# jcmgray/cotengra

Hardware: AMD Instinct MI355X
Metric: contracted FLOP/s (whole node), Sycamore n53 m20 sliced amplitude (higher is better)
Workload: dtype complex64; 1 GPU; Sycamore n53 m20 amplitude, sliced tree, one slice per step per GPU; network=examples/benchmarks/sycamore_n53_m20_s0_e0_pABCDCDAB.json, tree=sycamore_m20_native.json, width_log2=32, parallelism=slice-parallel x1, 1 RCCL reduce, arithmetic=fp16x2 stem pairs and long tiled steps + fp32 MFMA

## Files before the change

cotengra_amd/csrc/ctg_stem_impl.h:

```cpp
#pragma once
#include "ctg_common.h"

#include <cstdio>
#include <cstdlib>
#include <type_traits>


namespace ctg {

typedef float f32x16 __attribute__((ext_vector_type(16)));
typedef float f32x4 __attribute__((ext_vector_type(4)));

#ifdef CTG_STEM_BOUNDS
template <class AR>
__device__ unsigned long long ctg_stem_oob[2];
#endif

#ifdef CTG_STEM_TIMELINE
#define CTG_TL_TILES 256
template <class AR>
__device__ unsigned long long ctg_stem_tl[8][CTG_TL_TILES][6];
template <class AR>
__device__ int ctg_stem_tl_on;
#endif

namespace {

constexpr int SW = 8;
constexpr int BR1_CHUNKS = 2;

__device__ __forceinline__ f32x16 mfma(float a, float b, f32x16 c) {
    return __builtin_amdgcn_mfma_f32_32x32x2f32(a, b, c, 0, 0, 0);
}

__device__ __forceinline__ constexpr int rowmap(int t) { return (t & 3) + 8 * (t >> 2); }

__device__ __forceinline__ float flip(float v, unsigned mask) {
    return __builtin_bit_cast(float, __builtin_bit_cast(unsigned, v) ^ mask);
}

template <bool FRAG1>
__device__ __forceinline__ void load_b_planes(float* P, const c64* __restrict__ B, const int64_t* off, int K,
                                              int N, bool pack, int tid, bool vec = false) {
    const int LDB = K + 4;
    for (int e = tid; e < K * N; e += SW * 64) {
        const int k = e / N, n = e - k * N;
        const int h = vec ? (k >> 1) & 1 : k & 1;
        const int slot = vec ? (((k & 15) >> 2) << 1) | (k & 1) : (k & 15) >> 1;
        const int kp = FRAG1 ? (k & ~15) + h * 8 + slot : k;
        const c64 v = B[off[e]];
        P[n * LDB + kp] = v.re;
        P[(N + n) * LDB + kp] = v.im;
        if (pack) P[(2 * N + n) * LDB + kp] = -v.im;
    }
}


typedef __bf16 bf16x8 __attribute__((ext_vector_type(8)));
typedef unsigned u32x4 __attribute__((ext_vector_type(4)));
__device__ __forceinline__ constexpr int bf3_ta(int t) { return t < 3 ? 0 : (t == 5 ? 2 : 1); }
__device__ __forceinline__ constexpr int bf3_tb(int t) { return t == 1 || t == 4 ? 1 : (t == 2 ? 2 : 0); }

// ... 153 lines not shown
#endif

template <typename T>
__device__ __forceinline__ void settle(T& v) {
    asm volatile("" : "+v"(v));
}

#ifndef CTG_STEM_WS_DEPTH
#define CTG_STEM_WS_DEPTH 2
#endif
#ifndef CTG_STEM_DEPTH
#define CTG_STEM_DEPTH 2
#endif
template <class AR, bool PACK1, bool PACK2, int RT1_, int CS1, int NCH, int IT2_, bool BR1, int K2Q, bool VEC, bool BF3,
          bool RI2, bool ONE, int ITM, bool PACKM, bool XM, bool LM, bool WS>
__device__ __forceinline__ void stem2_body(const StemArgs& p) {
    constexpr bool TRI = ITM > 0;
    static_assert(!LM, "reserved (the limb intermediate was removed): kernel names stay 17 arguments long");
    static_assert(BF3 || !AR::fp16, "fp16 x 2: the 16-bit kernels only (its object has no fp32 products)");
    static_assert(!AR::fp16 || !TRI, "fp16 x 2: pairs and single steps");
    static_assert(!WS || (XM && !ONE && IT2_ > 0 && IT2_ <= 2 && (PACK1 || RT1_ == 1)), "specialised waves: a static 16-bit pair");
    constexpr int PW = WS ? 4 : SW;
    constexpr int RT1 = WS ? 2 * RT1_ : RT1_;
    constexpr int IT2 = WS ? 2 * IT2_ : IT2_;
    static_assert(!XM || (BF3 && !TRI && NCH > 0), "two-accumulator real part: bf16 x 3, static, no three-step tile");
    constexpr bool XM1 = XM && !PACK1 && !WS;
    constexpr bool XM2 = XM && !PACK2;
    static_assert(!TRI || (NCH > 0 && IT2 > 0 && !RI2 && !ONE && K2Q == 0), "three-step tile: static, X / Y form");
    static_assert(!ONE || (!PACK1 && !PACK2 && !RI2 && IT2 == 0 && K2Q == 0), "one step: >= 32 columns, nothing of step 2");
    static_assert(!PACK1 || CS1 == 1, "16 columns are one group");
    static_assert(!BR1 || NCH > 0, "B1 in registers needs the chunk count at compile time");
    static_assert(K2Q == 0 || PACK2 || IT2 == 1 || RI2, "B2 in registers: one column group per wave");
    static_assert(!RI2 || (!PACK2 && !BF3 && NCH > 0 && IT2 > 0), "row-interleaved step 2: fp32, >= 32 columns, static");
    constexpr int RTW = PW / CS1;
    constexpr bool STATIC = NCH > 0;
    extern __shared__ __attribute__((aligned(16))) char smem[];
    const int K1 = p.K1, N1 = p.N1, K2 = K2Q > 0 ? 4 * K2Q : p.K2, N2 = p.N2;
    const int LDB1 = K1 + 4, LDB2 = K2 + 4, LD2 = K2Q > 0 ? 4 * K2Q + 4 : p.ld2;
    const int PLANE = p.rows2 * LD2;
    const int KM = TRI ? p.KM : 0, NM = TRI ? p.NM : 0, LDM = TRI ? p.ldM : 0, LDBM = KM + 4;
    const int PLANEM = TRI ? p.rowsM * LDM : 0;
    const int PLANE1 = TRI ? PLANEM : PLANE;
    float* P1 = (float*)smem;
    float* PM = P1 + (PACK1 ? 3 : 2) * N1 * LDB1;
    float* P2 = PM + (TRI ? (PACKM ? 3 : 2) * NM * LDBM : 0);
    float* mid = P2 + (PACK2 ? 3 : 2) * N2 * LDB2;
    const int RP = 3 * LD2;
    auto ri_off = [&](int e) __attribute__((always_inline)) { return RI2 ? (e / LD2) * RP + e % LD2 : e; };
    int mid_floats = 2 * (PLANE > PLANEM ? PLANE : PLANEM);
    if constexpr (RI2) {
        mid_floats = 3 * PLANE;
        if constexpr (K2Q > 0) {
            mid = P2;
            const int p2f = 2 * N2 * LDB2;
            mid_floats = mid_floats > p2f ? mid_floats : p2f;
        }
    }
    const int ROW1 = bf3_row(K1, true), ROW2 = bf3_row(K2, false), ROWM = TRI ? bf3_row(KM, false) : 0;
    unsigned short* Q1 = (unsigned short*)smem;
    unsigned short* QM = Q1 + (PACK1 ? 3 : 2) * N1 * ROW1;
    unsigned short* Q2 = QM + (TRI ? (PACKM ? 3 : 2) * NM * ROWM : 0);
    if constexpr (BF3) mid = (float*)(Q2 + (PACK2 ? 3 : 2) * N2 * ROW2);
    int64_t* oc_s = (int64_t*)(mid + ((mid_floats + 1) & ~1));

    const int tid = threadIdx.x;
    const int lane = tid & 63;
    const int wave = __builtin_amdgcn_readfirstlane(tid >> 6);
    const int kk = lane >> 5;
    const int l31 = lane & 31;
    const bool producer = !WS || wave < PW;
    const int wave1 = WS ? (wave & (PW - 1)) : wave;
    const int wrt = wave1 / CS1;
    const int wcol = (wave1 % CS1) * 32;

    const int64_t z = (int64_t)p.z0 + blockIdx.y;
    const c64* __restrict__ A = (const c64*)p.A + (sload64(p.soffA + z * p.zsA) + z * p.zA);
    const c64* __restrict__ B1 = (const c64*)p.B1 + (sload64(p.soffB1 + z * p.zsB1) + z * p.zB1);
    const c64* __restrict__ B2 = (const c64*)p.B2 + (sload64(p.soffB2 + z * p.zsB2) + z * p.zB2);
    float* __restrict__ C = (float*)((c64*)p.C + (sload64(p.soffC + z * p.zsC) + z * p.zC));
    const c64* __restrict__ BM = TRI ? (const c64*)p.BM + (sload64(p.soffBM + z * p.zsBM) + z * p.zBM) : nullptr;

    int bf3_ex = 0;
    float* const bf3_red = (float*)(oc_s + (ONE ? N1 : N2));
    float h2_sa = 1.f;
    int h2_exa = 0;
    if constexpr (AR::fp16) {
        h2_exa = p.amax != nullptr ? h2_exponent_of(read_max(p.amax)) : 0;
        h2_exa = __builtin_amdgcn_readfirstlane(h2_exa);
        h2_sa = pow2f(-h2_exa);
    }
    float h2_st = 1.f;
    float h2_vmax = 0.f;
    if constexpr (BF3) {
        const int ex1 = bf3_operand_exponent<AR>(B1, p.b1_off, K1 * N1, tid, bf3_red);
        const int ex2 = ONE ? 0 : bf3_operand_exponent<AR>(B2, p.b2_off, K2 * N2, tid, bf3_red);
        int exm = 0;
        if constexpr (TRI) {
            exm = bf3_operand_exponent<AR>(BM, p.bm_off, KM * NM, tid, bf3_red);
            load_b_planes_bf3<AR, false>(QM, BM, p.bm_off, KM, NM, PACKM ? 3 : 2, tid, false, pow2f(-exm));
        }
        bf3_ex = ex1 + ex2 + exm;
        load_b_planes_bf3<AR, true>(Q1, B1, p.b1_off, K1, N1, PACK1 ? 3 : 2, tid, VEC, pow2f(-ex1));
        if constexpr (!ONE) load_b_planes_bf3<AR, false>(Q2, B2, p.b2_off, K2, N2, PACK2 ? 3 : 2, tid, false, pow2f(-ex2));
    } else {
        load_b_planes<true>(P1, B1, p.b1_off, K1, N1, PACK1, tid, VEC);
        if constexpr (!ONE) load_b_planes<false>(P2, B2, p.b2_off, K2, N2, PACK2, tid);
// ... 20 lines not shown
    }
    const unsigned sgn2 = kk ? 0x80000000u : 0u;
    const unsigned short* q1p;
    const unsigned short* q1q;
    const unsigned short* q2x;
    const unsigned short* q2y = nullptr;
    {
        const int h16 = l31 >> 4;
        if (PACK1) {
            q1p = Q1 + ((h16 ? 1 : 0) * N1 + (l31 & 15)) * ROW1 + kk * 24;
            q1q = Q1 + ((h16 ? 0 : 2) * N1 + (l31 & 15)) * ROW1 + kk * 24;
        } else {
            q1p = Q1 + (wcol + l31) * ROW1 + kk * 24;
            q1q = Q1 + (N1 + wcol + l31) * ROW1 + kk * 24;
        }
        if (PACK2) {
            const int plane = kk == 0 ? (h16 ? 1 : 0) : (h16 ? 0 : 2);
            q2x = Q2 + (plane * N2 + (l31 & 15)) * ROW2;
        } else {
            q2x = Q2 + ((kk ? 1 : 0) * N2 + l31) * ROW2;
            q2y = Q2 + ((kk ? 0 : 1) * N2 + l31) * ROW2;
        }
    }
    const float* b2x;
    const float* b2y = nullptr;
    if (PACK2) {
        const int n = l31 & 15, h = l31 >> 4;
        const int plane = kk == 0 ? (h ? 1 : 0) : (h ? 0 : 2);
        b2x = P2 + (plane * N2 + n) * LDB2;
    } else {
        b2x = P2 + ((kk ? 1 : 0) * N2 + l31) * LDB2;
        b2y = P2 + ((kk ? 0 : 1) * N2 + l31) * LDB2;
    }
    int mid_lane = 0;
    if constexpr (!ONE) {
        if (PACK1) mid_lane = ri_off((int)p.mid_col[l31 & 15]) + (l31 >> 4) * (RI2 ? LD2 : PLANE1) + ri_off((int)p.mid_row[4 * kk]);
        else mid_lane = ri_off((int)p.mid_col[wcol + l31]) + ri_off((int)p.mid_row[4 * kk]);
    }
    settle(mid_lane);
    int mid_o[4];
#pragma unroll
    for (int b = 0; b < 4; ++b) mid_o[b] = ONE ? 0 : ri_off((int)sload64(p.mid_row + (b < 2 ? 1 << b : 2 << b)));
    int mid_rt[RT1];
    int64_t one_rt[RT1];
#pragma unroll
    for (int m = 0; m < RT1; ++m) {
        mid_rt[m] = ONE ? 0 : __builtin_amdgcn_readfirstlane(ri_off((int)sload64(p.mid_row + 32 * (wrt + RTW * m))));
        one_rt[m] = ONE ? sload64(p.out_row + 32 * (wrt + RTW * m)) : 0;
    }
    const int64_t one_col = ONE ? p.out_col[wcol + l31] : 0;
    auto mid_t = [&](int t) __attribute__((always_inline)) {
        return ((t & 1) ? mid_o[0] : 0) + ((t & 2) ? mid_o[1] : 0) + ((t & 4) ? mid_o[2] : 0) + ((t & 8) ? mid_o[3] : 0);
    };
    int64_t out_lane = p.out_row[RI2 ? 2 * kk : 4 * kk];
    if (PACK2) out_lane += (l31 >> 4) ? p.out_row[1] : 0;
    settle(out_lane);
    int64_t out_o[4];
#pragma unroll
    for (int b = 0; b < 4; ++b) out_o[b] = sload64(p.out_row + (RI2 ? (b == 0 ? 1 : 2 << b) : (b < 2 ? 1 << b : 2 << b)));
    auto out_t = [&](int t) __attribute__((always_inline)) {
        return ((t & 1) ? out_o[0] : 0) + ((t & 2) ? out_o[1] : 0) + ((t & 4) ? out_o[2] : 0) + ((t & 8) ? out_o[3] : 0);
    };
    const int n_rtM = TRI ? p.rowsM >> 5 : 1;
    const unsigned short* qmx[TRI ? ITM : 1];
    const unsigned short* qmy[TRI ? ITM : 1];
    const float* bmx[TRI ? ITM : 1];
    const float* bmy[TRI ? ITM : 1];
    int m2_lane[TRI ? ITM : 1], m2_rt[TRI ? ITM : 1], am_row[TRI ? ITM : 1];
    int m2_o[4] = {0, 0, 0, 0};
    if constexpr (TRI) {
        const int h16 = l31 >> 4;
#pragma unroll
        for (int i = 0; i < ITM; ++i) {
            const int item = wave + SW * i;
            const int cg = item / n_rtM, rtm = item - cg * n_rtM;
            am_row[i] = (rtm * 32 + l31) * LDM;
            if (PACKM) {
                const int plane = kk == 0 ? (h16 ? 1 : 0) : (h16 ? 0 : 2);
                qmx[i] = QM + (plane * NM + (l31 & 15)) * ROWM;
                qmy[i] = nullptr;
                bmx[i] = PM + (plane * NM + (l31 & 15)) * LDBM;
// ... 20 lines not shown
    const int ri_cg = RI2 ? wave % p.ng2 : 0;
    const int ri_rt0 = RI2 ? wave / p.ng2 : 0;
    const int ri_rts = RI2 ? SW / p.ng2 : 0;
    const float* ri_b = P2 + (kk * N2 + ri_cg * 32 + l31) * LDB2;

    float alpha = 1.f, alpha2 = 1.f;
    {
        int e1 = bf3_ex < -126 ? -126 : (bf3_ex > 126 ? 126 : bf3_ex);
        int e2 = bf3_ex - e1;
        e2 = e2 < -126 ? -126 : (e2 > 126 ? 126 : e2);
        if (p.facA != nullptr) {
            const double f = (*p.facA) * (*p.facB1) * (*p.facB2) * (TRI ? *p.facBM : 1.0);
            alpha = (f == 0.0 && p.check_zero) ? 0.f : (float)(1.0 / f * (BF3 ? exp2((double)e1) : 1.0));
        } else if (BF3 && bf3_ex != 0) {
            alpha = pow2f(e1);
        }
        if (BF3 && e2 != 0) alpha2 = pow2f(e2);
    }
    const int h2_e0 = bf3_ex + h2_exa;
    auto h2_set_alpha = [&](int et) __attribute__((always_inline)) {
        const int E = h2_e0 + et;
        const int e1 = E < -126 ? -126 : (E > 126 ? 126 : E);
        int e2 = E - e1;
        e2 = e2 < -126 ? -126 : (e2 > 126 ? 126 : e2);
        alpha = pow2f(e1);
        alpha2 = pow2f(e2);
    };
    if constexpr (AR::fp16) h2_set_alpha(0);
    const bool scaled = AR::fp16 ? true : __builtin_amdgcn_readfirstlane(alpha != 1.f || alpha2 != 1.f);
    __syncthreads();

    f32x4 b1r[BR1 && !BF3 ? NCH * 2 : 1][2];
    f32x4 b2r[K2Q > 0 && !BF3 ? K2Q : 1][PACK2 ? 1 : 2];
    bf16x8 b1r3[BR1 && BF3 ? NCH : 1][3][2];
    if constexpr (BR1 && BF3) {
#pragma unroll
        for (int c = 0; c < NCH; ++c)
#pragma unroll
            for (int q = 0; q < 3; ++q) {
                b1r3[c][q][0] = *(const bf16x8*)(q1p + c * 48 + q * 8);
                b1r3[c][q][1] = *(const bf16x8*)(q1q + c * 48 + q * 8);
            }
    }
    if constexpr (BR1 && !BF3) {
#pragma unroll
        for (int q = 0; q < NCH * 2; ++q) {
            b1r[q][0] = *(const f32x4*)(b1p + (q >> 1) * 16 + (q & 1) * 4);
            b1r[q][1] = *(const f32x4*)(b1q + (q >> 1) * 16 + (q & 1) * 4);
        }
    }
    if constexpr (K2Q > 0 && RI2) {
#pragma unroll
        for (int q = 0; q < K2Q; ++q) b2r[q][0] = *(const f32x4*)(ri_b + 4 * q);
    }
    if constexpr (K2Q > 0 && !BF3 && !RI2) {
        const int cg0 = PACK2 ? 0 : wave / (p.rows2 >> 5);
#pragma unroll
        for (int q = 0; q < K2Q; ++q) {
            b2r[q][0] = *(const f32x4*)(b2x + cg0 * 32 * LDB2 + 4 * q);
            if (!PACK2) {
                b2r[q][1] = *(const f32x4*)(b2y + cg0 * 32 * LDB2 + 4 * q);
#pragma unroll
                for (int t = 0; t < 4; ++t) b2r[q][0][t] = flip(b2r[q][0][t], sgn2);
            }
        }
    }
    const int nch = STATIC ? NCH : (K1 >> 4);
    const int n_rt2 = p.rows2 >> 5;
    const int n_items = n_rt2 * p.ng2;
    const int64_t n_tiles = p.n_tiles;
    const int64_t tile0 = blockIdx.x, tile_step = gridDim.x;
    const int64_t my_tiles = (n_tiles - tile0 + tile_step - 1) / tile_step;
    const int64_t last_tile = tile0 + (my_tiles - 1) * tile_step;

    constexpr int GD = WS ? CTG_STEM_WS_DEPTH : ((NCH > 0 && CTG_STEM_DEPTH == 4 && ((RT1 * NCH) & 1) == 0) ? 4 : 2);
    c64 regs[GD][8];
    int64_t ig = tile0;
    int im = 0, ic = 0;
    int64_t pend0 = 0, pend1 = 0, pend2 = 0, pend3 = 0;
    bool pend_live = false;
    auto prep = [&](auto always_tag) __attribute__((always_inline)) {
        constexpr bool ALWAYS = decltype(always_tag)::value;
        pend_live = ALWAYS || ig < n_tiles;
        if (pend_live) {
            const int64_t g = ALWAYS ? (ig < last_tile ? ig : last_tile) : ig;
            const int64_t gh = g >> p.g_lo_shift, gl = g & (p.g_lo - 1);
            pend0 = sload64(p.gA_hi + uniform64(gh));
            pend1 = sload64(p.gA_lo + uniform64(gl));
            pend2 = sload64(p.rt_a + (wrt + RTW * im));
            pend3 = sload64(p.chunk_a + ic);
            if (++ic == nch) {
                ic = 0;
                if (++im == RT1) {
                    im = 0;
                    ig += tile_step;
                }
            }
        }
    };
    auto fire2 = [&](c64 (&r)[8], int q, int64_t base, auto always_tag) __attribute__((always_inline)) {
        if (decltype(always_tag)::value || pend_live) {
            if constexpr (XM) {
                typedef const __attribute__((address_space(1))) char* gptr;
                uint64_t u0 = (uint64_t)A + ((uint64_t)(base + kj[2 * q]) << 3);
                uint64_t u1 = (uint64_t)A + ((uint64_t)(base + kj[2 * q + 1]) << 3);
                asm volatile("" : "+s"(u0), "+s"(u1));
                settle(a_lane);
                const unsigned al = a_lane;
                if (VEC) {
                    const f32x4 v = *(const __attribute__((address_space(1))) f32x4*)((gptr)u0 + al);
                    r[2 * q] = c64{v[0], v[1]};
                    r[2 * q + 1] = c64{v[2], v[3]};
                } else {
                    typedef float f32x2 __attribute__((ext_vector_type(2)));
                    const f32x2 v0 = *(const __attribute__((address_space(1))) f32x2*)((gptr)u0 + al);
                    const f32x2 v1 = *(const __attribute__((address_space(1))) f32x2*)((gptr)u1 + al);
                    r[2 * q] = c64{v0[0], v0[1]};
                    r[2 * q + 1] = c64{v1[0], v1[1]};
                }
                return;
            }
            const char* sb = (const char*)(A + (base + kj[2 * q]));
#ifdef CTG_STEM_BOUNDS
            {
                const uint64_t lim = (uint64_t)p.a_elems * 8;
                const uint64_t o0 = (uint64_t)(sb + a_lane - (const char*)A);
// ... 43 lines not shown
        }
#endif
        *(float2*)q = v;
    };
    auto drain = [&](int lo, int hi, auto set_tag, auto scaled_tag) __attribute__((always_inline)) {
        constexpr int SET = decltype(set_tag)::value < NSET ? decltype(set_tag)::value : 0;
#pragma unroll
        for (int i = lo; i < hi; ++i) {
            if constexpr (RI2) {
                float2 v;
                v.x = cr[SET][i >> 3][2 * (i & 7)];
                v.y = cr[SET][i >> 3][2 * (i & 7) + 1];
                if constexpr (decltype(scaled_tag)::value) {
                    v.x = v.x * alpha * alpha2;
                    v.y = v.y * alpha * alpha2;
                }
                store2(pdst + 2 * out_t(i), v);
            } else {
                store2(pdst + 2 * out_t(PACK2 ? 2 * i : i), pv[i]);
            }
        }
    };
    auto consume = [&](c64 (&r)[8], int m, int ch, auto always_tag, auto drain_tag, auto scaled_tag)
                       __attribute__((always_inline)) {
        constexpr bool DRAIN = decltype(drain_tag)::value >= 0;
        const int64_t base = pend0 + pend1 + pend2 + pend3;
        if constexpr (BF3) {
            float re[8], im[8];
#pragma unroll
            for (int j = 0; j < 8; ++j) {
                re[j] = r[j].re;
                im[j] = r[j].im;
            }
            bf16x8 r3[3], i3[3], n3[3], bp3[3], bq3[3];
            AR::split(re, r3, h2_sa);
            AR::split(im, i3, h2_sa);
            __builtin_amdgcn_sched_barrier(0);
#pragma unroll
            for (int q = 0; q < 4; ++q) fire2(r, q, base, always_tag);
#pragma unroll
            for (int q = 0; q < 3; ++q) {
                if (!PACK1 && !XM1) n3[q] = __builtin_bit_cast(bf16x8, __builtin_bit_cast(u32x4, i3[q]) ^ 0x80008000u);
                if constexpr (BR1) {
                    bp3[q] = b1r3[ch][q][0];
                    bq3[q] = b1r3[ch][q][1];
                } else {
                    bp3[q] = *(const bf16x8*)(q1p + ch * 48 + q * 8);
                    bq3[q] = *(const bf16x8*)(q1q + ch * 48 + q * 8);
                }
            }
            __builtin_amdgcn_sched_barrier(0);
            const bool fresh = XM && STATIC && ch == 0;
            f32x16 zero16;
#pragma unroll
            for (int u = 0; u < 16; ++u) zero16[u] = 0.f;
#pragma unroll
            for (int t = 0; t < 6; t += AR::t_step(t)) {
                const int ta = bf3_ta(t), tb = bf3_tb(t);
                if (PACK1) {
                    ax[m] = AR::mfma(r3[ta], bp3[tb], (fresh && t == 0) ? zero16 : ax[m]);
                    ax[m] = AR::mfma(i3[ta], bq3[tb], ax[m]);
                } else if constexpr (XM1) {
                    ax[m] = AR::mfma(r3[ta], bp3[tb], (fresh && t == 0) ? zero16 : ax[m]);
                    ay[m] = AR::mfma(r3[ta], bq3[tb], (fresh && t == 0) ? zero16 : ay[m]);
                    axm[m] = AR::mfma(i3[ta], bq3[tb], (fresh && t == 0) ? zero16 : axm[m]);
                    ay[m] = AR::mfma(i3[ta], bp3[tb], ay[m]);
                } else {
                    ax[m] = AR::mfma(r3[ta], bp3[tb], (fresh && t == 0) ? zero16 : ax[m]);
                    ay[m] = AR::mfma(r3[ta], bq3[tb], (fresh && t == 0) ? zero16 : ay[m]);
                    ax[m] = AR::mfma(n3[ta], bq3[tb], ax[m]);
                    ay[m] = AR::mfma(i3[ta], bp3[tb], ay[m]);
                }
                __builtin_amdgcn_sched_barrier(0);
                if constexpr (DRAIN)
                    drain(AR::t_index(t) * NST / AR::products, (AR::t_index(t) + 1) * NST / AR::products, drain_tag, scaled_tag);
            }
            __builtin_amdgcn_sched_barrier(0);
            prep(always_tag);
            __builtin_amdgcn_sched_barrier(0);
            return;
        }
        f32x4 bp[2], bq[2];
        if constexpr (BR1) {
            bp[0] = b1r[ch * 2][0];
            bp[1] = b1r[ch * 2 + 1][0];
            bq[0] = b1r[ch * 2][1];
            bq[1] = b1r[ch * 2 + 1][1];
        } else {
            bp[0] = *(const f32x4*)(b1p + ch * 16);
            bq[0] = *(const f32x4*)(b1q + ch * 16);
            bp[1] = *(const f32x4*)(b1p + ch * 16 + 4);
            bq[1] = *(const f32x4*)(b1q + ch * 16 + 4);
        }
#pragma unroll
        for (int j = 0; j < 8; ++j) {
            const float re = r[j].re, im = r[j].im;
            const float p_ = bp[j >> 2][j & 3], q_ = bq[j >> 2][j & 3];
            __builtin_amdgcn_sched_barrier(0);
            if (PACK1) {
                ax[m] = mfma(re, p_, ax[m]);
                ax[m] = mfma(im, q_, ax[m]);
            } else {
                ax[m] = mfma(re, p_, ax[m]);
                ay[m] = mfma(re, q_, ay[m]);
                ax[m] = mfma(flip(im, sgn), q_, ax[m]);
                ay[m] = mfma(im, p_, ay[m]);
            }
            __builtin_amdgcn_sched_barrier(0);
            if (j & 1) fire2(r, j >> 1, base, always_tag);
            if constexpr (DRAIN) drain(j * NST / 8, (j + 1) * NST / 8, drain_tag, scaled_tag);
        }
        __builtin_amdgcn_sched_barrier(0);
        prep(always_tag);
        __builtin_amdgcn_sched_barrier(0);
    };
    auto zero_acc = [&](int m) __attribute__((always_inline)) {
        if constexpr (XM && STATIC) return;
#pragma unroll
        for (int t = 0; t < 16; ++t) {
            ax[m][t] = 0.f;
            if (!PACK1) ay[m][t] = 0.f;
            if constexpr (XM1) axm[m][t] = 0.f;
        }
    };
    auto scatter = [&]() __attribute__((always_inline)) {
#pragma unroll
        for (int m = 0; m < RT1; ++m) {
            float* dst = mid + (mid_lane + mid_rt[m]);
#pragma unroll
            for (int t = 0; t < 16; ++t) {
                dst[mid_t(t)] = XM1 ? ax[m][t] - axm[m][t] : ax[m][t];
                if constexpr (RI2) {
                    if constexpr (PACK1) {
                        if (l31 >> 4) dst[LD2 + mid_t(t)] = -ax[m][t];
                    } else {
                        dst[LD2 + mid_t(t)] = ay[m][t];
                        dst[2 * LD2 + mid_t(t)] = -ay[m][t];
                    }
                } else {
                    if (!PACK1) dst[PLANE1 + mid_t(t)] = ay[m][t];
                }
            }
        }
    };
    auto item_row = [&](int item, int64_t c_tile) __attribute__((always_inline)) -> int64_t {
        const int cg = item / n_rt2, rt2 = item - cg * n_rt2;
        int64_t c_row = c_tile + sload64(p.out_row + 32 * rt2);
        asm volatile("" : "+s"(c_row));
        return c_row;
    };
    auto item2r = [&](int rt2, int64_t c_row, auto set_tag, auto prev_tag, auto scaled_tag) __attribute__((always_inline)) {
        constexpr int SET = decltype(set_tag)::value;
        constexpr bool DRAIN = decltype(prev_tag)::value >= 0;
        const float* a0p = mid + ri_plane + (rt2 * 32 + (l31 >> 1)) * RP;
        const float* a1p = a0p + 16 * RP;
        const int64_t c_col = oc_s[ri_cg * 32 + l31];
        f32x4 a0[2], a1[2], bq[2];
        a0[0] = *(const f32x4*)(a0p);
        a1[0] = *(const f32x4*)(a1p);
        constexpr int NQ = K2Q > 0 ? K2Q : 1;
        if constexpr (K2Q > 0) {
// ... 192 lines not shown
            constexpr bool SC = decltype(scaled_tag)::value;
            pdst = C + 2 * (c_row + out_lane + c_col);
            if (PACK2) {
                const bool hi = (l31 >> 4) != 0;
#pragma unroll
                for (int t = 0; t < 16; t += 2) {
                    const float mine = hi ? cx[t] : cx[t + 1];
                    const float got = __builtin_bit_cast(
                        float, __builtin_amdgcn_ds_swizzle(__builtin_bit_cast(int, mine), 0x401F));
                    float2 v;
                    v.x = hi ? got : cx[t];
                    v.y = hi ? cx[t + 1] : got;
                    if (SC) {
                        v.x = v.x * alpha * alpha2;
                        v.y = v.y * alpha * alpha2;
                    }
                    if constexpr (BF3) h2_vmax = fmaxf(h2_vmax, fmaxf(fabsf(v.x), fabsf(v.y)));
                    pv[t >> 1] = v;
                }
            } else {
#pragma unroll
                for (int t = 0; t < 16; ++t) {
                    float2 v;
                    const float xr = XM2 ? cx[t] - cxm[t] : cx[t];
                    v.x = SC ? xr * alpha * alpha2 : xr;
                    v.y = SC ? cy[t] * alpha * alpha2 : cy[t];
                    if constexpr (BF3) h2_vmax = fmaxf(h2_vmax, fmaxf(fabsf(v.x), fabsf(v.y)));
                    pv[t] = v;
                }
            }
            if constexpr (!decltype(defer_tag)::value) drain(0, NST, std::integral_constant<int, 0>{}, scaled_tag);
        }
    };
    f32x16 mx[TRI ? ITM : 1], my[TRI ? ITM : 1];
    auto item_mid = [&](auto ii) __attribute__((always_inline)) {
        constexpr int I = decltype(ii)::value;
        f32x16 cx, cy;
#pragma unroll
        for (int t = 0; t < 16; ++t) {
            cx[t] = 0.f;
            cy[t] = 0.f;
        }
        const float* a_base = mid + kk * PLANEM + am_row[I];
        if constexpr (BF3) {
            for (int kb = 0; kb < (KM >> 3); ++kb) {
                const f32x4 lo = *(const f32x4*)(a_base + 8 * kb), hi = *(const f32x4*)(a_base + 8 * kb + 4);
                const float a8[8] = {lo[0], lo[1], lo[2], lo[3], hi[0], hi[1], hi[2], hi[3]};
                bf16x8 a3[3], ax3[3], bx3[3], by3[3];
                AR::split(a8, a3);
#pragma unroll
                for (int q = 0; q < 3; ++q) {
                    ax3[q] = PACKM ? a3[q]
                                   : __builtin_bit_cast(bf16x8, __builtin_bit_cast(u32x4, a3[q]) ^ (sgn2 | (sgn2 >> 16)));
                    bx3[q] = *(const bf16x8*)(qmx[I] + kb * 24 + q * 8);
                    if (!PACKM) by3[q] = *(const bf16x8*)(qmy[I] + kb * 24 + q * 8);
                }
#pragma unroll
                for (int t = 0; t < 6; t += AR::t_step(t)) {
                    cx = AR::mfma(ax3[bf3_ta(t)], bx3[bf3_tb(t)], cx);
                    if (!PACKM) cy = AR::mfma(a3[bf3_ta(t)], by3[bf3_tb(t)], cy);
                }
            }
        } else {
            const int nq = KM >> 2;
            f32x4 af[2], bx[2], by[2];
            af[0] = *(const f32x4*)(a_base);
// ... 51 lines not shown
            float mx = 0.f;
#pragma unroll
            for (int m = 0; m < RT1; ++m)
#pragma unroll
                for (int t = 0; t < 16; ++t) {
                    const float xr = XM1 ? ax[m][t] - axm[m][t] : ax[m][t];
                    mx = fmaxf(mx, fabsf(xr));
                    if (!PACK1) mx = fmaxf(mx, fabsf(ay[m][t]));
                }
#pragma unroll
            for (int o = 32; o > 0; o >>= 1) mx = fmaxf(mx, __shfl_xor(mx, o));
            if (lane == 0) bf3_red[h2_par * 8 + wave1] = mx;
            if constexpr (WS) h2_par ^= 1;
        }
    };
    auto h2_consume = [&]() __attribute__((always_inline)) {
        if constexpr (AR::fp16 && !ONE) {
            float mx = bf3_red[h2_par * 8];
#pragma unroll
            for (int w = 1; w < PW; ++w) mx = fmaxf(mx, bf3_red[h2_par * 8 + w]);
            const int et = __builtin_amdgcn_readfirstlane(h2_exponent_of(mx));
            h2_st = pow2f(-et);
            h2_set_alpha(et);
            h2_par ^= 1;
        }
    };
    auto tile_c = [&](int64_t g) __attribute__((always_inline)) -> int64_t {
        const int64_t gh = g >> p.g_lo_shift, gl = g & (p.g_lo - 1);
        return sload64(p.gC_hi + uniform64(gh)) + sload64(p.gC_lo + uniform64(gl));
    };

    auto run = [&](auto scaled_tag) __attribute__((always_inline)) {
    if constexpr (WS) {
        constexpr int NT = RT1 * NCH;
        constexpr int U = (NT % GD == 0) ? 1 : ((2 * NT) % GD == 0 ? 2 : 4);
        static_assert((U * NT) % GD == 0, "a pass of U tiles returns to gather set 0");
        auto step1 = [&](auto slot0_tag) __attribute__((always_inline)) {
            constexpr int SLOT0 = decltype(slot0_tag)::value;
            static_for<0, RT1>([&](auto mi) __attribute__((always_inline)) {
                constexpr int M = decltype(mi)::value;
                static_for<0, NCH>([&](auto ci) __attribute__((always_inline)) {
                    constexpr int CH = decltype(ci)::value;
                    consume(regs[(SLOT0 + M * NCH + CH) & (GD - 1)], M, CH, std::true_type{}, std::integral_constant<int, -1>{}, scaled_tag);
                });
            });
        };
        auto step2 = [&](int64_t gc) __attribute__((always_inline)) {
            const int64_t c_tile = tile_c(gc);
            int64_t c_rows[IT2];
            static_for<0, IT2>([&](auto ii) __attribute__((always_inline)) {
                c_rows[decltype(ii)::value] = item_row(wave1 + PW * decltype(ii)::value, c_tile);
            });
            static_for<0, IT2>([&](auto ii) __attribute__((always_inline)) {
                constexpr int I = decltype(ii)::value;
                item2(wave1 + PW * I, c_rows[I], scaled_tag, std::integral_constant<bool, (I > 0)>{}, std::true_type{});
            });
        };
        if (producer) {
            static_for<0, GD>([&](auto gi) __attribute__((always_inline)) { issue(regs[decltype(gi)::value], std::true_type{}); });
            prep(std::true_type{});
            step1(std::integral_constant<int, 0>{});
            for (int64_t t = 0; t < my_tiles; t += U) {
                static_for<0, U>([&](auto ui) __attribute__((always_inline)) {
                    constexpr int UI = decltype(ui)::value;
                    if (t + UI < my_tiles) {
                        h2_publish();
                        __syncthreads();
                        scatter();
                        __syncthreads();
                        if (t + UI + 1 < my_tiles) step1(std::integral_constant<int, ((UI + 1) * NT) & (GD - 1)>{});
                    }
                });
            }
        } else {
            for (int64_t t = 0; t < my_tiles; ++t) {
                __syncthreads();
                if (t > 0) drain(0, NST, std::integral_constant<int, 0>{}, scaled_tag);
                __syncthreads();
                h2_consume();
                step2(tile0 + t * tile_step);
            }
            drain(0, NST, std::integral_constant<int, 0>{}, scaled_tag);
// ... 496 lines not shown
    if (form == 3 && items == 2 * SW && p.N2 >= 32) form = 1;
    if (items >= 4 * SW) form = 0;
    return form;
}

template <class AR>
static void stem_kernel_name(const StemArgs& p, char* buf, size_t n) {
    const StemShape s = stem2_shape(p);
    const char* const kn = AR::kernel_name;
    auto tf = [](bool b) { return b ? "true" : "false"; };
    if (p.tri) {
        const Stem3Shape t = stem3_shape(p);
        snprintf(buf, n, "%s<%s,%s,%d,%d,%d,%d,%s,0,%s,%s,false,false,%d,%s>", kn, tf(t.p1), tf(t.p2), t.rt1, t.cs1,
                 t.nch, t.it2, tf(t.nch <= BR1_CHUNKS), tf(t.vec), tf(stem_wants_16bit(p)), t.itm, tf(t.pm));
        return;
    }
    if (p.one) {
        const bool st = stem1_static(s), b3 = stem2_bf3(p);
        if (st && b3)
            snprintf(buf, n, "%s<false,false,%d,%d,%d,0,%s,0,%s,true,false,true,0,false,true,false>", kn, s.rt1, s.cs1,
                     s.nch, tf(s.nch <= BR1_CHUNKS), tf(s.vec));
        else
            snprintf(buf, n, "%s<false,false,%d,%d,%d,0,%s,0,%s,%s,false,true>", kn, s.rt1, s.cs1, st ? s.nch : 0,
                     tf(st && (b3 ? s.nch <= BR1_CHUNKS : p.K1 <= 64)), tf(s.vec), tf(b3));
        return;
    }
    if (stem2_bf3(p)) {
        const int form = stem2_bf3_form<AR>(p);
        if (form == 0)
            snprintf(buf, n, "%s<%s,%s,%d,%d,%d,%d,%s,0,%s,true,false,false>", kn, tf(s.p1), tf(s.p2), s.rt1, s.cs1,
                     s.nch, s.it2, tf(s.nch <= BR1_CHUNKS), tf(s.vec));
        else
            snprintf(buf, n, "%s<%s,%s,%d,%d,%d,%d,%s,0,%s,true,false,false,0,false,true,false,%s>", kn, tf(s.p1), tf(s.p2),
                     s.rt1, s.cs1, s.nch, s.it2, tf(s.nch <= BR1_CHUNKS), tf(s.vec), tf(form >= 3));
    }
    else if (stem2_variant(p))
        snprintf(buf, n, "%s<%s,%s,%d,%d,%d,%d,%s,%d,%s,false,%s,false>", kn, tf(s.p1), tf(s.p2), s.rt1, s.cs1, s.nch,
                 s.it2, tf(s.br1), s.k2q, tf(s.vec), tf(s.ri2));
    else
        snprintf(buf, n, "%s<%s,%s,%d,%d,0,0,false,0,%s,false,false,false>", kn, tf(s.p1), tf(s.p2), s.rt1, s.cs1,
                 tf(s.vec));
}

static bool stem_uses_16bit(const StemArgs& p) { return !p.tri && stem2_supported_shape(p) && stem2_bf3(p); }

template <class AR>
static hipError_t launch_stem(const StemArgs& p, hipStream_t stream) {
    if (!stem2_supported_shape(p)) return hipErrorInvalidValue;
    if constexpr (AR::fp16) {
        if (!stem_uses_16bit(p)) return hipErrorInvalidValue;
    } else {
        if (p.tri) {
            const Stem3Shape t = stem3_shape(p);
            const bool b3 = stem_wants_16bit(p);
#define CTG_STEM_GO3T(A, M, B, R, CS, NC, IM, IT, V)                                                                  \
    if (t.p1 == A && t.pm == M && t.p2 == B && t.rt1 == R && t.cs1 == CS && t.nch == NC && t.itm == IM && t.it2 == IT && \
        t.vec == V)                                                                                                   \
        return b3 ? launch_stem3_t<A, M, B, R, CS, NC, IM, IT, V, true>(p, stream)                                    \
                  : launch_stem3_t<A, M, B, R, CS, NC, IM, IT, V, false>(p, stream);
            CTG_STEM_TRI(CTG_STEM_GO3T)
#undef CTG_STEM_GO3T
            return hipErrorInvalidValue;
        }
    }
    if (p.one) {
        const StemShape s = stem2_shape(p, true);
        const bool b3 = stem2_bf3(p);
        if (stem1_static(s)) {
#define CTG_STEM_GO1(R, CS, NC, V)                                                                            \
    if (s.rt1 == R && s.cs1 == CS && s.nch == NC && s.vec == V) {                                             \
        if (b3) return launch_stem1_t<AR, R, CS, NC, (NC <= BR1_CHUNKS), V, true>(p, stream);                 \
        if constexpr (!AR::fp16) return launch_stem1_t<AR, R, CS, NC, (NC <= 4), V, false>(p, stream);        \
    }
            CTG_STEM_ONE(CTG_STEM_GO1)
#undef CTG_STEM_GO1
        }
        if constexpr (!AR::fp16) {
#define CTG_STEM_CASE1(R, CS)                                                               \
    if (s.rt1 == R && s.cs1 == CS)                                                          \
        return s.vec ? launch_stem1_t<AR, R, CS, 0, false, true, false>(p, stream)          \
                     : launch_stem1_t<AR, R, CS, 0, false, false, false>(p, stream);
            CTG_STEM_CASE1(1, 1) CTG_STEM_CASE1(2, 1) CTG_STEM_CASE1(1, 2) CTG_STEM_CASE1(2, 2)
            CTG_STEM_CASE1(1, 4) CTG_STEM_CASE1(2, 4)
#undef CTG_STEM_CASE1
        }
        return hipErrorInvalidValue;
    }
    if (stem2_bf3(p)) {
        const StemShape s = stem2_shape(p, true);
        const int form = stem2_bf3_form<AR>(p);
#define CTG_STEM_GO3(P1, P2, R, CS, NC, IT, V)                                                                           \
    if (s.p1 == P1 && s.p2 == P2 && s.rt1 == R && s.cs1 == CS && s.nch == NC && s.it2 == IT && s.vec == V) {             \
        if constexpr (AR::max_form >= 3 && IT <= 2 && (P1 || R == 1) && (P2 || IT < 2)) {                                \
            if (form == 3)                                                                                               \
                return launch_stem2_t<AR, P1, P2, R, CS, NC, IT, (NC <= BR1_CHUNKS), 0, V, true, false, true, true>(p, stream);  \
        }                                                                                                                \
        if constexpr (IT < 4) {                                                                                          \
            if (form == 1)                                                                                               \
                return launch_stem2_t<AR, P1, P2, R, CS, NC, IT, (NC <= BR1_CHUNKS), 0, V, true, false, true, false>(p, stream); \
        } else {                                                                                                         \
            if (form == 0) return launch_stem2_t<AR, P1, P2, R, CS, NC, IT, (NC <= BR1_CHUNKS), 0, V, true>(p, stream);  \
        }                                                                                                                \
        return hipErrorInvalidValue;                                                                                     \
    }
        CTG_STEM_GEO(CTG_STEM_GO3)
#undef CTG_STEM_GO3
    }
    if constexpr (!AR::fp16) {
        const StemShape s = stem2_shape(p);
        if (stem2_variant(p)) {
#define CTG_STEM_GO(P1, P2, R, CS, NC, IT, B1, KQ, V, RI)                                              \
    if (s.p1 == P1 && s.p2 == P2 && s.rt1 == R && s.cs1 == CS && s.nch == NC && s.it2 == IT && s.br1 == B1 && \
        s.k2q == KQ && s.vec == V && s.ri2 == RI)                                                      \
        return launch_stem2_t<AR, P1, P2, R, CS, NC, IT, B1, KQ, V, false, RI>(p, stream);
            CTG_STEM_INST(CTG_STEM_GO)
#undef CTG_STEM_GO
        }
#define CTG_STEM_CASE(P1, P2, R, CS)                                                                    \
    if (s.p1 == P1 && s.p2 == P2 && s.rt1 == R && s.cs1 == CS)                                          \
        return s.vec ? launch_stem2_t<AR, P1, P2, R, CS, 0, 0, false, 0, true>(p, stream)               \
                     : launch_stem2_t<AR, P1, P2, R, CS, 0, 0, false, 0, false>(p, stream);
#define CTG_STEM_CASES(P2)             \
    CTG_STEM_CASE(true, P2, 1, 1)      \
    CTG_STEM_CASE(true, P2, 2, 1)      \
    CTG_STEM_CASE(false, P2, 1, 1)     \
    CTG_STEM_CASE(false, P2, 2, 1)     \
    CTG_STEM_CASE(false, P2, 1, 2)     \
    CTG_STEM_CASE(false, P2, 2, 2)     \
// ... 13 lines not shown
```

Measured before the change: 161400 billion FLOP/s.

## Share A fragments across column groups in specialised-wave stem and add K-chunked step-2 path

In the warp-specialised 16-bit stem pair, when several column groups exist each wave now covers all column groups of a row tile. The split A fragment is reused across column groups instead of being recomputed per wave, and B1 register residency is sized to match. A new step-2 routine (item2k) handles two column groups per wave with the A fragments kept in registers and B chunks double-buffered. The aim is to cut redundant A splitting and LDS reads, at the cost of more registers per wave and possible occupancy or spill pressure.

```diff
diff --git a/cotengra_amd/csrc/ctg_stem_impl.h b/cotengra_amd/csrc/ctg_stem_impl.h
--- a/cotengra_amd/csrc/ctg_stem_impl.h
+++ b/cotengra_amd/csrc/ctg_stem_impl.h
@@ -28,6 +28,7 @@
 
 constexpr int SW = 8;
 constexpr int BR1_CHUNKS = 2;
+constexpr bool stem_br1_ws(int cs1, int nch) { return (cs1 == 2 ? 2 : 1) * nch <= BR1_CHUNKS; }
 
 __device__ __forceinline__ f32x16 mfma(float a, float b, f32x16 c) {
     return __builtin_amdgcn_mfma_f32_32x32x2f32(a, b, c, 0, 0, 0);
@@ -247,7 +248,10 @@
     static_assert(!BR1 || NCH > 0, "B1 in registers needs the chunk count at compile time");
     static_assert(K2Q == 0 || PACK2 || IT2 == 1 || RI2, "B2 in registers: one column group per wave");
     static_assert(!RI2 || (!PACK2 && !BF3 && NCH > 0 && IT2 > 0), "row-interleaved step 2: fp32, >= 32 columns, static");
-    constexpr int RTW = PW / CS1;
+    constexpr bool SH1 = WS && CS1 > 1 && RT1 % CS1 == 0;
+    constexpr int CG1 = SH1 ? CS1 : 1;
+    constexpr int RR1 = RT1 / CG1;
+    constexpr int RTW = SH1 ? PW : PW / CS1;
     constexpr bool STATIC = NCH > 0;
     extern __shared__ __attribute__((aligned(16))) char smem[];
     const int K1 = p.K1, N1 = p.N1, K2 = K2Q > 0 ? 4 * K2Q : p.K2, N2 = p.N2;
@@ -285,8 +289,8 @@
     const int l31 = lane & 31;
     const bool producer = !WS || wave < PW;
     const int wave1 = WS ? (wave & (PW - 1)) : wave;
-    const int wrt = wave1 / CS1;
-    const int wcol = (wave1 % CS1) * 32;
+    const int wrt = SH1 ? wave1 : wave1 / CS1;
+    const int wcol = SH1 ? 0 : (wave1 % CS1) * 32;
 
     const int64_t z = (int64_t)p.z0 + blockIdx.y;
     const c64* __restrict__ A = (const c64*)p.A + (sload64(p.soffA + z * p.zsA) + z * p.zA);
@@ -373,12 +377,16 @@
         b2x = P2 + ((kk ? 1 : 0) * N2 + l31) * LDB2;
         b2y = P2 + ((kk ? 0 : 1) * N2 + l31) * LDB2;
     }
-    int mid_lane = 0;
-    if constexpr (!ONE) {
-        if (PACK1) mid_lane = ri_off((int)p.mid_col[l31 & 15]) + (l31 >> 4) * (RI2 ? LD2 : PLANE1) + ri_off((int)p.mid_row[4 * kk]);
-        else mid_lane = ri_off((int)p.mid_col[wcol + l31]) + ri_off((int)p.mid_row[4 * kk]);
-    }
-    settle(mid_lane);
+    int mid_lane[CG1];
+#pragma unroll
+    for (int cg = 0; cg < CG1; ++cg) {
+        mid_lane[cg] = 0;
+        if constexpr (!ONE) {
+            if (PACK1) mid_lane[cg] = ri_off((int)p.mid_col[l31 & 15]) + (l31 >> 4) * (RI2 ? LD2 : PLANE1) + ri_off((int)p.mid_row[4 * kk]);
+            else mid_lane[cg] = ri_off((int)p.mid_col[wcol + 32 * cg + l31]) + ri_off((int)p.mid_row[4 * kk]);
+        }
+        settle(mid_lane[cg]);
+    }
     int mid_o[4];
 #pragma unroll
     for (int b = 0; b < 4; ++b) mid_o[b] = ONE ? 0 : ri_off((int)sload64(p.mid_row + (b < 2 ? 1 << b : 2 << b)));
@@ -386,8 +394,8 @@
     int64_t one_rt[RT1];
 #pragma unroll
     for (int m = 0; m < RT1; ++m) {
-        mid_rt[m] = ONE ? 0 : __builtin_amdgcn_readfirstlane(ri_off((int)sload64(p.mid_row + 32 * (wrt + RTW * m))));
-        one_rt[m] = ONE ? sload64(p.out_row + 32 * (wrt + RTW * m)) : 0;
+        mid_rt[m] = ONE ? 0 : __builtin_amdgcn_readfirstlane(ri_off((int)sload64(p.mid_row + 32 * (wrt + RTW * (m / CG1)))));
+        one_rt[m] = ONE ? sload64(p.out_row + 32 * (wrt + RTW * (m / CG1))) : 0;
     }
     const int64_t one_col = ONE ? p.out_col[wcol + l31] : 0;
     auto mid_t = [&](int t) __attribute__((always_inline)) {
@@ -474,15 +482,18 @@
 
     f32x4 b1r[BR1 && !BF3 ? NCH * 2 : 1][2];
     f32x4 b2r[K2Q > 0 && !BF3 ? K2Q : 1][PACK2 ? 1 : 2];
-    bf16x8 b1r3[BR1 && BF3 ? NCH : 1][3][2];
+    bf16x8 b1r3[CG1][BR1 && BF3 ? NCH : 1][3][2];
+    const int q1cg = 32 * ROW1;
     if constexpr (BR1 && BF3) {
 #pragma unroll
-        for (int c = 0; c < NCH; ++c)
-#pragma unroll
-            for (int q = 0; q < 3; ++q) {
-                b1r3[c][q][0] = *(const bf16x8*)(q1p + c * 48 + q * 8);
-                b1r3[c][q][1] = *(const bf16x8*)(q1q + c * 48 + q * 8);
-            }
+        for (int cg = 0; cg < CG1; ++cg)
+#pragma unroll
+            for (int c = 0; c < NCH; ++c)
+#pragma unroll
+                for (int q = 0; q < 3; ++q) {
+                    b1r3[cg][c][q][0] = *(const bf16x8*)(q1p + cg * q1cg + c * 48 + q * 8);
+                    b1r3[cg][c][q][1] = *(const bf16x8*)(q1q + cg * q1cg + c * 48 + q * 8);
+                }
     }
     if constexpr (BR1 && !BF3) {
 #pragma unroll
@@ -533,7 +544,7 @@
             pend3 = sload64(p.chunk_a + ic);
             if (++ic == nch) {
                 ic = 0;
-                if (++im == RT1) {
+                if (++im == RR1) {
                     im = 0;
                     ig += tile_step;
                 }
@@ -643,7 +654,7 @@
                 re[j] = r[j].re;
                 im[j] = r[j].im;
             }
-            bf16x8 r3[3], i3[3], n3[3], bp3[3], bq3[3];
+            bf16x8 r3[3], i3[3], n3[3], bp3[CG1][3], bq3[CG1][3];
             AR::split(re, r3, h2_sa);
             AR::split(im, i3, h2_sa);
             __builtin_amdgcn_sched_barrier(0);
@@ -652,12 +663,15 @@
 #pragma unroll
             for (int q = 0; q < 3; ++q) {
                 if (!PACK1 && !XM1) n3[q] = __builtin_bit_cast(bf16x8, __builtin_bit_cast(u32x4, i3[q]) ^ 0x80008000u);
-                if constexpr (BR1) {
-                    bp3[q] = b1r3[ch][q][0];
-                    bq3[q] = b1r3[ch][q][1];
-                } else {
-                    bp3[q] = *(const bf16x8*)(q1p + ch * 48 + q * 8);
-                    bq3[q] = *(const bf16x8*)(q1q + ch * 48 + q * 8);
+#pragma unroll
+                for (int cg = 0; cg < CG1; ++cg) {
+                    if constexpr (BR1) {
+                        bp3[cg][q] = b1r3[cg][ch][q][0];
+                        bq3[cg][q] = b1r3[cg][ch][q][1];
+                    } else {
+                        bp3[cg][q] = *(const bf16x8*)(q1p + cg * q1cg + ch * 48 + q * 8);
+                        bq3[cg][q] = *(const bf16x8*)(q1q + cg * q1cg + ch * 48 + q * 8);
+                    }
                 }
             }
             __builtin_amdgcn_sched_barrier(0);
@@ -669,18 +683,26 @@
             for (int t = 0; t < 6; t += AR::t_step(t)) {
                 const int ta = bf3_ta(t), tb = bf3_tb(t);
                 if (PACK1) {
-                    ax[m] = AR::mfma(r3[ta], bp3[tb], (fresh && t == 0) ? zero16 : ax[m]);
-                    ax[m] = AR::mfma(i3[ta], bq3[tb], ax[m]);
+                    ax[m] = AR::mfma(r3[ta], bp3[0][tb], (fresh && t == 0) ? zero16 : ax[m]);
+                    ax[m] = AR::mfma(i3[ta], bq3[0][tb], ax[m]);
                 } else if constexpr (XM1) {
-                    ax[m] = AR::mfma(r3[ta], bp3[tb], (fresh && t == 0) ? zero16 : ax[m]);
-                    ay[m] = AR::mfma(r3[ta], bq3[tb], (fresh && t == 0) ? zero16 : ay[m]);
-                    axm[m] = AR::mfma(i3[ta], bq3[tb], (fresh && t == 0) ? zero16 : axm[m]);
-                    ay[m] = AR::mfma(i3[ta], bp3[tb], ay[m]);
+                    ax[m] = AR::mfma(r3[ta], bp3[0][tb], (fresh && t == 0) ? zero16 : ax[m]);
+                    ay[m] = AR::mfma(r3[ta], bq3[0][tb], (fresh && t == 0) ? zero16 : ay[m]);
+                    axm[m] = AR::mfma(i3[ta], bq3[0][tb], (fresh && t == 0) ? zero16 : axm[m]);
+                    ay[m] = AR::mfma(i3[ta], bp3[0][tb], ay[m]);
                 } else {
-                    ax[m] = AR::mfma(r3[ta], bp3[tb], (fresh && t == 0) ? zero16 : ax[m]);
-                    ay[m] = AR::mfma(r3[ta], bq3[tb], (fresh && t == 0) ? zero16 : ay[m]);
-                    ax[m] = AR::mfma(n3[ta], bq3[tb], ax[m]);
-                    ay[m] = AR::mfma(i3[ta], bp3[tb], ay[m]);
+#pragma unroll
+                    for (int cg = 0; cg < CG1; ++cg) {
+                        const int u = m * CG1 + cg;
+                        ax[u] = AR::mfma(r3[ta], bp3[cg][tb], (fresh && t == 0) ? zero16 : ax[u]);
+                        ay[u] = AR::mfma(r3[ta], bq3[cg][tb], (fresh && t == 0) ? zero16 : ay[u]);
+                    }
+#pragma unroll
+                    for (int cg = 0; cg < CG1; ++cg) {
+                        const int u = m * CG1 + cg;
+                        ax[u] = AR::mfma(n3[ta], bq3[cg][tb], ax[u]);
+                        ay[u] = AR::mfma(i3[ta], bp3[cg][tb], ay[u]);
+                    }
                 }
                 __builtin_amdgcn_sched_barrier(0);
                 if constexpr (DRAIN)
@@ -737,7 +759,7 @@
     auto scatter = [&]() __attribute__((always_inline)) {
 #pragma unroll
         for (int m = 0; m < RT1; ++m) {
-            float* dst = mid + (mid_lane + mid_rt[m]);
+            float* dst = mid + (mid_lane[m % CG1] + mid_rt[m]);
 #pragma unroll
             for (int t = 0; t < 16; ++t) {
                 dst[mid_t(t)] = XM1 ? ax[m][t] - axm[m][t] : ax[m][t];
@@ -996,6 +1018,76 @@
             if constexpr (!decltype(defer_tag)::value) drain(0, NST, std::integral_constant<int, 0>{}, scaled_tag);
         }
     };
+    auto item2k = [&](auto nc_tag, int item0, int64_t c_row, auto scaled_tag) __attribute__((always_inline)) {
+        constexpr int NC = decltype(nc_tag)::value;
+        constexpr bool SC = decltype(scaled_tag)::value;
+        const int cg0 = item0 / n_rt2, rt2 = item0 - cg0 * n_rt2;
+        const int cgs = PW / n_rt2;
+        const int bI = N2 * ROW2;
+        const float* aRf = mid + (rt2 * 32 + l31) * LD2 + kk * 8;
+        struct FragA { bf16x8 ar[3], ai[3]; };
+        struct FragB { bf16x8 br[3], bi[3]; };
+        FragA AK[NC];
+        FragB BF[2];
+        f32x16 cx, cy, cxm;
+        auto load_a = [&](FragA& F, int c) __attribute__((always_inline)) {
+            const f32x4 r0 = *(const f32x4*)(aRf + 16 * c), r1 = *(const f32x4*)(aRf + 16 * c + 4);
+            const f32x4 i0 = *(const f32x4*)(aRf + PLANE + 16 * c), i1 = *(const f32x4*)(aRf + PLANE + 16 * c + 4);
+            const float re8[8] = {r0[0], r0[1], r0[2], r0[3], r1[0], r1[1], r1[2], r1[3]};
+            const float im8[8] = {i0[0], i0[1], i0[2], i0[3], i1[0], i1[1], i1[2], i1[3]};
+            AR::split(re8, F.ar, h2_st);
+            AR::split(im8, F.ai, h2_st);
+        };
+        auto load_b = [&](FragB& F, const unsigned short* bR, int c) __attribute__((always_inline)) {
+#pragma unroll
+            for (int q = 0; q < 3; ++q) {
+                F.br[q] = *(const bf16x8*)(bR + c * 48 + q * 8);
+                F.bi[q] = *(const bf16x8*)(bR + bI + c * 48 + q * 8);
+            }
+        };
+        auto mul = [&](const FragA& A_, const FragB& B_, bool first) __attribute__((always_inline)) {
+            f32x16 zero16;
+#pragma unroll
+            for (int u = 0; u < 16; ++u) zero16[u] = 0.f;
+#pragma unroll
+            for (int t = 0; t < 6; t += AR::t_step(t)) {
+                const int ta = bf3_ta(t), tb = bf3_tb(t);
+                cx = AR::mfma(A_.ar[ta], B_.br[tb], (first && t == 0) ? zero16 : cx);
+                cy = AR::mfma(A_.ar[ta], B_.bi[tb], (first && t == 0) ? zero16 : cy);
+                cxm = AR::mfma(A_.ai[ta], B_.bi[tb], (first && t == 0) ? zero16 : cxm);
+                cy = AR::mfma(A_.ai[ta], B_.br[tb], cy);
+            }
+        };
+        auto emit = [&](int cg) __attribute__((always_inline)) {
+            pdst = C + 2 * (c_row + out_lane + oc_s[cg * 32 + l31]);
+#pragma unroll
+            for (int t = 0; t < 16; ++t) {
+                float2 v;
+                const float xr = cx[t] - cxm[t];
+                v.x = SC ? xr * alpha * alpha2 : xr;
+                v.y = SC ? cy[t] * alpha * alpha2 : cy[t];
+                h2_vmax = fmaxf(h2_vmax, fmaxf(fabsf(v.x), fabsf(v.y)));
+                pv[t] = v;
+            }
+        };
+        static_for<0, 2>([&](auto gi) __attribute__((always_inline)) {
+            constexpr int G = decltype(gi)::value;
+            const int cg = cg0 + G * cgs;
+            const unsigned short* bR = Q2 + (cg * 32 + l31) * ROW2 + kk * 24;
+            if constexpr (G == 1) drain(0, NST, std::integral_constant<int, 0>{}, scaled_tag);
+            if constexpr (G == 0) load_a(AK[0], 0);
+            load_b(BF[0], bR, 0);
+            static_for<0, NC>([&](auto ci) __attribute__((always_inline)) {
+                constexpr int CH = decltype(ci)::value;
+                if constexpr (CH + 1 < NC) {
+                    if constexpr (G == 0) load_a(AK[CH + 1], CH + 1);
+                    load_b(BF[(CH + 1) & 1], bR, CH + 1);
+                }
+                mul(AK[CH], BF[CH & 1], CH == 0);
+            });
+            emit(cg);
+        });
+    };
     f32x16 mx[TRI ? ITM : 1], my[TRI ? ITM : 1];
     auto item_mid = [&](auto ii) __attribute__((always_inline)) {
         constexpr int I = decltype(ii)::value;
@@ -1113,12 +1205,12 @@
 
     auto run = [&](auto scaled_tag) __attribute__((always_inline)) {
     if constexpr (WS) {
-        constexpr int NT = RT1 * NCH;
+        constexpr int NT = RR1 * NCH;
         constexpr int U = (NT % GD == 0) ? 1 : ((2 * NT) % GD == 0 ? 2 : 4);
         static_assert((U * NT) % GD == 0, "a pass of U tiles returns to gather set 0");
         auto step1 = [&](auto slot0_tag) __attribute__((always_inline)) {
             constexpr int SLOT0 = decltype(slot0_tag)::value;
-            static_for<0, RT1>([&](auto mi) __attribute__((always_inline)) {
+            static_for<0, RR1>([&](auto mi) __attribute__((always_inline)) {
                 constexpr int M = decltype(mi)::value;
                 static_for<0, NCH>([&](auto ci) __attribute__((always_inline)) {
                     constexpr int CH = decltype(ci)::value;
@@ -1129,6 +1221,19 @@
         auto step2 = [&](int64_t gc) __attribute__((always_inline)) {
             const int64_t c_tile = tile_c(gc);
             int64_t c_rows[IT2];
+            if constexpr (IT2 == 2 && XM2) {
+                if (n_rt2 <= PW) {
+                    const int nc = K2 >> 4;
+                    if (nc == 4) {
+                        item2k(std::integral_constant<int, 4>{}, wave1, item_row(wave1, c_tile), scaled_tag);
+                        return;
+                    }
+                    if (nc == 2) {
+                        item2k(std::integral_constant<int, 2>{}, wave1, item_row(wave1, c_tile), scaled_tag);
+                        return;
+                    }
+                }
+            }
             static_for<0, IT2>([&](auto ii) __attribute__((always_inline)) {
                 c_rows[decltype(ii)::value] = item_row(wave1 + PW * decltype(ii)::value, c_tile);
             });
@@ -1691,7 +1796,8 @@
                      s.nch, s.it2, tf(s.nch <= BR1_CHUNKS), tf(s.vec));
         else
             snprintf(buf, n, "%s<%s,%s,%d,%d,%d,%d,%s,0,%s,true,false,false,0,false,true,false,%s>", kn, tf(s.p1), tf(s.p2),
-                     s.rt1, s.cs1, s.nch, s.it2, tf(s.nch <= BR1_CHUNKS), tf(s.vec), tf(form >= 3));
+                     s.rt1, s.cs1, s.nch, s.it2, tf(form >= 3 ? stem_br1_ws(s.cs1, s.nch) : s.nch <= BR1_CHUNKS), tf(s.vec),
+                     tf(form >= 3));
     }
     else if (stem2_variant(p))
         snprintf(buf, n, "%s<%s,%s,%d,%d,%d,%d,%s,%d,%s,false,%s,false>", kn, tf(s.p1), tf(s.p2), s.rt1, s.cs1, s.nch,
@@ -1752,7 +1858,7 @@
     if (s.p1 == P1 && s.p2 == P2 && s.rt1 == R && s.cs1 == CS && s.nch == NC && s.it2 == IT && s.vec == V) {             \
         if constexpr (AR::max_form >= 3 && IT <= 2 && (P1 || R == 1) && (P2 || IT < 2)) {                                \
             if (form == 3)                                                                                               \
-                return launch_stem2_t<AR, P1, P2, R, CS, NC, IT, (NC <= BR1_CHUNKS), 0, V, true, false, true, true>(p, stream);  \
+                return launch_stem2_t<AR, P1, P2, R, CS, NC, IT, stem_br1_ws(CS, NC), 0, V, true, false, true, true>(p, stream);  \
         }                                                                                                                \
         if constexpr (IT < 4) {                                                                                          \
             if (form == 1)                                                                                               \
```

Result: faster. 166500 billion FLOP/s, median of 6 (+3.1%).
